# rajabala/Volumetric-Particles-For-Unity

Measured on AMD Instinct MI355X. Metric: Mvoxels/s filled + Msamples/s raymarched, 32³×32³ grid @1080p, higher is better.
Workload: dtype f32 compute / f16 voxel storage

## Files before the change

### volumetric-particles-for-unity_amd/csrc/api.cpp

```cpp
#include <cmath>
#include <cstdarg>
#include <cstdio>
#include <cstdlib>
#include <cstring>
#include <new>

#include "vpfx_internal.h"

thread_local std::string g_vp_create_error;

int vp_fail(vp_ctx* c, int code, const char* fmt, ...)
{
    char buf[512];
    va_list ap;
    va_start(ap, fmt);
    vsnprintf(buf, sizeof buf, fmt, ap);
    va_end(ap);
    if (c) c->err = buf; else g_vp_create_error = buf;
    return code;
}

namespace {

template <typename T>
// ... 224 lines not shown
    hipError_t e = hipGetDeviceCount(&ndev);
    if (e != hipSuccess || ndev < 1)
        return vp_fail(nullptr, VP_ERR_NO_DEVICE, "vp_create: no HIP device (%s); libvpfx has no CPU fallback",
                       e != hipSuccess ? hipGetErrorString(e) : "device count 0");
    int dev = cfg->device;
    if (dev < 0) { if (hipGetDevice(&dev) != hipSuccess) dev = 0; }
    if (dev >= ndev) return vp_fail(nullptr, VP_ERR_BAD_ARG, "vp_create: device %d of %d", dev, ndev);

    c = new (std::nothrow) vp_ctx();
    if (!c) return vp_fail(nullptr, VP_ERR_OOM, "vp_create: host allocation failed");
    c->cfg = *cfg;
    c->device = dev;
    if (cfg->multi_flags & VP_MULTI_TEST_HOOKS) { const char* hook = getenv("VPFX_TEST_CHAIN_TIMEOUT"); c->test_chain_timeout = hook && hook[0] == '1'; }
    { const char* sw = getenv("VPFX_RM_NO_SPACE_SKIP"); c->rm_space_skip = !sw ? 0 : sw[0] == '1' ? -1 : sw[0] == '0' ? 1 : 0; }
    { const char* sw = getenv("VPFX_RM_NO_BOX_CLIP"); c->rm_box_clip = !sw ? 0 : sw[0] == '1' ? -1 : sw[0] == '0' ? 1 : 0; }
#if VPFX_AB
    { const char* sw = getenv("VPFX_NO_ZPROFILE"); c->no_zprofile = sw && sw[0] == '1'; }
    { const char* sw = getenv("VPFX_RM_FLAT"); c->rm_flat = sw && sw[0] == '1'; }
    { const char* sw = getenv("VPFX_RM_XCD_AFFINE"); c->rm_xcd_affine = sw && sw[0] == '1'; }
#endif
    c->n3 = (size_t)cfg->num_mv[0] * cfg->num_mv[1] * cfg->num_mv[2];
    memset(c->L, 0, sizeof c->L); c->L[0] = c->L[5] = c->L[10] = c->L[15] = 1.f;
    c->h_mvPos = (float*)malloc(c->n3 * 3 * sizeof(float));
    int rc = VP_OK;
    auto fail = [&](int code) { g_vp_create_error = c->err; vp_destroy_single(c); return code; };
    if (!c->h_mvPos) { c->err = "vp_create: host allocation failed"; return fail(VP_ERR_OOM); }
    hl_build_grid(c);
    if ((rc = ensure_device(c))) return fail(rc);
    if (hipDeviceGetAttribute(&c->num_cus, hipDeviceAttributeMultiprocessorCount, dev) != hipSuccess || c->num_cus < 1) c->num_cus = 256;
    const size_t nxy = (size_t)cfg->num_mv[0] * cfg->num_mv[1];
    if ((rc = dev_alloc(c, &c->d_mvPos, c->n3 * 3)) || (rc = dev_alloc(c, &c->d_count, c->n3)) ||
        (rc = dev_alloc(c, &c->d_offsets, c->n3 + 1)) || (rc = dev_alloc(c, &c->d_cursor, c->n3)) ||
        (rc = dev_alloc(c, &c->d_brick_index, c->n3)) || (rc = dev_alloc(c, &c->d_occ_list, c->n3)) ||
        (rc = dev_alloc(c, &c->d_onecol, 2)) || (rc = dev_alloc(c, &c->d_work_counter, 1)) || (rc = dev_alloc(c, &c->d_meta, 1)) ||
        (rc = dev_alloc(c, &c->d_ord, c->n3)) || (rc = dev_alloc(c, &c->d_colcount, nxy)) || (rc = dev_alloc(c, &c->d_chain, lightmap_elems(c))) ||
        (rc = dev_alloc(c, (int4**)&c->d_scan_totals, (c->n3 + 1023) / 1024 + 1)) ||
        (rc = dev_alloc(c, &c->d_lightmap, lightmap_elems(c))) || (rc = dev_alloc(c, &c->d_rank, nxy)) ||
        (rc = dev_alloc(c, &c->d_image, image_elems(c))) || (rc = dev_alloc(c, &c->d_samples, 1)) ||
        (rc = dev_alloc(c, &c->d_zsamples, (size_t)VPFX_ZPROF_COPIES * cfg->num_mv[2])) ||
        (rc = dev_alloc(c, &c->d_tile_order, (size_t)rm_order_ints(rm_num_super_tiles(cfg->width, cfg->height)) + rm_num_super_tiles(cfg->width, cfg->height) + 8)))
        return fail(rc);
#if VPFX_AB
    {
        const int sgx = rm_super_tiles_x(cfg->width), sgy = rm_super_tiles_y(cfg->height), ns = sgx * sgy;
        int side = 1; while (side < sgx || side < sgy) side <<= 1;
        std::vector<int> curve; curve.reserve(ns);
        for (long long d = 0; d < (long long)side * side; ++d) {
            long long tt = d; int x = 0, y = 0;
// ... 24 lines not shown
}

VP_EXPORT void vp_destroy(vp_ctx* c)
{
    if (!c) return;
    if (c->multi) { multi_destroy(c); return; }
    vp_destroy_single(c);
}

void vp_destroy_single(vp_ctx* c)
{
    if (!c) return;
    (void)hipSetDevice(c->device);
    if (c->stream) (void)hipStreamSynchronize(c->stream); else (void)hipDeviceSynchronize();
    void* dev[] = {c->d_mvPos, c->d_raw, c->d_ws, c->d_rec, c->d_count, c->d_offsets, c->d_cursor, c->d_brick_index,
                   c->d_occ_list, c->d_ids_tmp, c->d_ids, c->d_onecol, c->d_work_counter, c->d_ord, c->d_colcount, c->d_chain, c->d_cube_u8, c->d_meta, c->d_scan_totals, c->d_bricks, c->d_dens_ao,
                   c->d_lightmap, c->d_cubequads, c->d_depthmap, c->d_occluders, c->d_mvtrans, c->d_brick_hit, c->d_rank, c->d_tile_order, c->d_tile_curve, c->d_image, c->d_scene_depth, c->d_samples, c->d_zsamples, c->d_cellinfo, c->d_occmask, c->d_slab_rect, c->d_mvbox[0], c->d_mvbox[1]};
    for (void* p : dev) if (p) (void)hipFree(p);
    mesh_free_all(c);
    device_emitters_orphan_all(c);
    particle_queries_free(c);
    if (c->h_chain_err) (void)hipHostFree(c->h_chain_err);
    if (c->h_meta_host) (void)hipHostFree(c->h_meta_host);
    if (c->copy_stream) { (void)hipStreamSynchronize(c->copy_stream); (void)hipStreamDestroy(c->copy_stream); }
    if (c->ev_image_ready) (void)hipEventDestroy(c->ev_image_ready);
    if (c->ev_image_copied) (void)hipEventDestroy(c->ev_image_copied);
    for (int s = 0; s < 4; ++s) for (int j = 0; j < 2; ++j) if (c->ev[s][j]) (void)hipEventDestroy(c->ev[s][j]);
    free(c->h_mvPos);
    delete c;
}

// ... 817 lines not shown
```

### volumetric-particles-for-unity_amd/csrc/bin.hip

```cpp
#include "vpfx_internal.h"
#include "mv_box.h"

#include <chrono>

namespace {

__device__ __forceinline__ float rd_f32(const uint8_t* p)
{
    uint32_t v = (uint32_t)p[0] | ((uint32_t)p[1] << 8) | ((uint32_t)p[2] << 16) | ((uint32_t)p[3] << 24);
    return __uint_as_float(v);
}

__device__ __forceinline__ void sincos_deg(float deg, float& s, float& c)
{
    const float k = rintf(deg * (1.0f / 90.0f));
    const float r = fmaf(-90.0f, k, deg);
    const float x = r * 0.017453292519943295f;
    const float z = x * x;
    const float sp = fmaf(fmaf(fmaf(-1.9515295891e-4f, z, 8.3321608736e-3f), z, -1.6666654611e-1f), z * x, x);
    const float cp = fmaf(fmaf(fmaf(2.443315711809948e-5f, z, -1.388731625493765e-3f), z, 4.166664568298827e-2f),
                          z * z, fmaf(-0.5f, z, 1.0f));
    switch (((int)k) & 3) {
    case 0: s = sp; c = cp; break;
    case 1: s = cp; c = -sp; break;
// ... 35 lines not shown
    for (int k = 0; k < 3; ++k) {
        const float rx = R[0 * 3 + k] * inv, ry = R[1 * 3 + k] * inv, rz = R[2 * 3 + k] * inv;
        out[k * 4 + 0] = rx; out[k * 4 + 1] = ry; out[k * 4 + 2] = rz;
        out[k * 4 + 3] = -((rx * wx + ry * wy) + rz * wz);
    }
    out[12] = life / life0;
    out[13] = 0.f; out[14] = 0.f; out[15] = 0.f;
    float4* dst = reinterpret_cast<float4*>(rec + 16 * (size_t)p);
    dst[0] = make_float4(out[0], out[1], out[2], out[3]);
    dst[1] = make_float4(out[4], out[5], out[6], out[7]);
    dst[2] = make_float4(out[8], out[9], out[10], out[11]);
    dst[3] = make_float4(out[12], out[13], out[14], out[15]);
}

#define BIN_LANES 32
template <int MODE>
__global__ void __launch_bounds__(256)
k_bin(const float4* __restrict__ ws4, int P, GridConsts g, const float* __restrict__ mvPos,
      int* __restrict__ count_or_cursor, const int* __restrict__ offsets, int* __restrict__ ids, float* __restrict__ rec,
      const DevMeta* __restrict__ ahead_meta, int ahead_cap)
{
    const long long t = (long long)blockIdx.x * 256 + threadIdx.x;
    const int p = (int)(t / BIN_LANES), sub = (int)(t % BIN_LANES);
    if (p >= P) return;
    if (MODE == 1 && ahead_meta && (unsigned)ahead_meta->pairs > (unsigned)ahead_cap) return;
    const float4 w = ws4[p];
    if (MODE == 0 && sub == 0) {
        float* r = rec + 16 * (size_t)p;
        const float dx = g.fwd[0] * g.one, dy = g.fwd[1] * g.one, dz = g.fwd[2] * g.one;
        r[13] = fmaf(r[2], dz, fmaf(r[1], dy, r[0] * dx));
        r[14] = fmaf(r[6], dz, fmaf(r[5], dy, r[4] * dx));
        r[15] = fmaf(r[10], dz, fmaf(r[9], dy, r[8] * dx));
    }
    if (!(fabsf(w.x) < INFINITY && fabsf(w.y) < INFINITY && fabsf(w.z) < INFINITY && fabsf(w.w) < INFINITY)) return;
    const float lx = ((g.Linv[0] * w.x + g.Linv[1] * w.y) + g.Linv[2] * w.z) + g.Linv[3];
    const float ly = ((g.Linv[4] * w.x + g.Linv[5] * w.y) + g.Linv[6] * w.z) + g.Linv[7];
    const float lz = ((g.Linv[8] * w.x + g.Linv[9] * w.y) + g.Linv[10] * w.z) + g.Linv[11];
    const float pix = (lx - g.lsO[0]) / g.s + (float)g.Nx * 0.5f;
    const float piy = (ly - g.lsO[1]) / g.s + (float)g.Ny * 0.5f;
    const float piz = (lz - g.lsO[2]) / g.s + (float)g.Nz * 0.5f;
    const float fe = (float)(int)rintf((w.w / 2.0f) / g.s);
    const int x0 = (int)fmaxf(0.f, pix - fe), x1 = (int)fminf((float)(g.Nx - 1), pix + fe);
    const int y0 = (int)fmaxf(0.f, piy - fe), y1 = (int)fminf((float)(g.Ny - 1), piy + fe);
    int z0 = (int)fmaxf(0.f, piz - fe), z1 = (int)fminf((float)(g.Nz - 1), piz + fe);
    if (MODE != 2) { z0 = max(z0, g.z0); z1 = min(z1, g.z1 - 1); }
    const float r = (w.w / 2.0f) / g.sb;
    const int nx = x1 - x0 + 1, ny = y1 - y0 + 1, nz = z1 - z0 + 1;
    if (nx <= 0 || ny <= 0 || nz <= 0) return;
    const int ncand = nx * ny * nz;
    for (int ci = sub; ci < ncand; ci += BIN_LANES) {
                const int xx = x0 + ci % nx, yy = y0 + (ci / nx) % ny, zz = z0 + ci / (nx * ny);
                const int mi = (zz * g.Ny + yy) * g.Nx + xx;
                const float mx = mvPos[3 * mi], my = mvPos[3 * mi + 1], mz = mvPos[3 * mi + 2];
                float r2 = r * r;
#pragma unroll
                for (int k = 0; k < 3; ++k) {
                    const float a = g.rowsb[k * 3], bq = g.rowsb[k * 3 + 1], cq = g.rowsb[k * 3 + 2];
                    const float t = -((a * mx + bq * my) + cq * mz);
                    const float m = ((a * w.x + bq * w.y) + cq * w.z) + t;
                    if (m < -0.5f) { const float d = m - (-0.5f); r2 -= d * d; }
                    else if (m > 0.5f) { const float d = m - 0.5f; r2 -= d * d; }
                }
                if (r2 > 0.f) {
                    if (MODE == 2) atomicAdd(&count_or_cursor[zz], 1);
                    else if (MODE == 0) atomicAdd(&count_or_cursor[mi], 1);
                    else { const int slot = atomicAdd(&count_or_cursor[mi], 1); ids[offsets[mi] + slot] = p; }
                }
            }
}

#define SCAN_TILE 1024
#define SCAN_DIRECT_TILES 4096
struct TileTotals { long long pairs; int occ, mx; };

__device__ __forceinline__ void block_scan3(long long& a, int& b, int& m, long long* sh )
{
    const int lane = threadIdx.x & 63, wv = threadIdx.x >> 6;
#pragma unroll
    for (int d = 1; d < 64; d <<= 1) {
        const long long ua = __shfl_up(a, d);
        const int ub = __shfl_up(b, d), um = __shfl_up(m, d);
        if (lane >= d) { a += ua; b += ub; m = max(m, um); }
    }
// ... 34 lines not shown
        const int t = base + threadIdx.x;
        const TileTotals tt = t < ntiles ? totals[t] : TileTotals{0, 0, 0};
        long long a = tt.pairs;
        int b = tt.occ, m = tt.mx;
        block_scan3(a, b, m, sh);
        const long long ca = s_carry[0];
        const int cb = (int)s_carry[1], cm = (int)s_carry[2];
        if (t < ntiles) totals[t] = TileTotals{ca + a - tt.pairs, cb + b - tt.occ, 0};
        __syncthreads();
        if (threadIdx.x == SCAN_TILE - 1) { s_carry[0] = ca + a; s_carry[1] = cb + b; s_carry[2] = max(cm, m); }
        __syncthreads();
    }
    if (threadIdx.x == 0) totals[ntiles] = TileTotals{s_carry[0], (int)s_carry[1], (int)s_carry[2]};
}

__device__ __forceinline__ void publish_totals(DevMeta* host_meta, const DevMeta& r, int seq)
{
    *host_meta = r;
    __hip_atomic_store(reinterpret_cast<int*>(host_meta + 1), seq, __ATOMIC_RELEASE, __HIP_MEMORY_SCOPE_SYSTEM);
}

__global__ void __launch_bounds__(SCAN_TILE)
k_scan_write(const int* __restrict__ count, int n3, int nxy, int z0, int z1, const TileTotals* __restrict__ totals, int ntiles,
             int prefixed, int* __restrict__ offsets, int* __restrict__ brick_index, int* __restrict__ occ_list, int* __restrict__ cursor,
             DevMeta* __restrict__ meta, DevMeta* __restrict__ host_meta, int seq, uint2* __restrict__ mvbox)
{
    __shared__ long long sh[48];
    __shared__ long long s_base[3];
    if (prefixed) {
        if (threadIdx.x == 0) { s_base[0] = totals[blockIdx.x].pairs; s_base[1] = totals[blockIdx.x].occ; s_base[2] = totals[ntiles].mx; }
    } else {
        long long pa = 0;
        int pb = 0, pm = 0;
        for (int t = threadIdx.x; t < ntiles; t += SCAN_TILE) {
            const TileTotals tt = totals[t];
            if (t < (int)blockIdx.x) { pa += tt.pairs; pb += tt.occ; }
            pm = max(pm, tt.mx);
        }
        block_scan3(pa, pb, pm, sh);
        if (threadIdx.x == SCAN_TILE - 1) { s_base[0] = pa; s_base[1] = pb; s_base[2] = pm; }
    }
    __syncthreads();
    const long long base_pairs = s_base[0];
// ... 6 lines not shown
    int b = occ ? 1 : 0, m = cnt;
    block_scan3(a, b, m, sh);
    if (i < n3) {
        offsets[i] = (int)(base_pairs + a - cnt);
        cursor[i] = 0;
        const int slot = base_occ + b - (occ ? 1 : 0);
        brick_index[i] = occ ? slot : -1;
        if (occ) occ_list[slot] = i;
        else mvbox[i] = make_uint2(VPFX_MVBOX_EMPTY_X, VPFX_MVBOX_EMPTY_Y);
    }
    if ((int)blockIdx.x == ntiles - 1 && threadIdx.x == SCAN_TILE - 1) {
        const long long total = base_pairs + a;
        offsets[n3] = (int)total;
        const DevMeta r{base_occ + b, total > 2147483647LL ? -1 : (int)total, gmax, 0};
        *meta = r;
        publish_totals(host_meta, r, seq);
    }
}

__global__ void __launch_bounds__(SCAN_TILE)
k_scan_small(const int* __restrict__ count, int n3, int nxy, int z0, int z1, int* __restrict__ offsets, int* __restrict__ brick_index,
             int* __restrict__ occ_list, int* __restrict__ cursor, int* __restrict__ ord, int* __restrict__ colcount,
             DevMeta* __restrict__ meta, DevMeta* __restrict__ host_meta, int seq, uint2* __restrict__ mvbox)
{
    __shared__ long long sh[48];
    __shared__ unsigned char s_occ[SCAN_TILE];
    const int i = threadIdx.x;
    const int cnt = i < n3 ? count[i] : 0;
    const int zz = i / nxy;
    const bool occ = cnt != 0 && zz >= z0 && zz < z1;
    s_occ[i] = occ ? 1 : 0;
// ... 14 lines not shown
        } else mvbox[i] = make_uint2(VPFX_MVBOX_EMPTY_X, VPFX_MVBOX_EMPTY_Y);
        if (i < nxy) {
            int n = 0;
            for (int z = z0; z < z1; ++z) n += s_occ[z * nxy + i];
            colcount[i] = n;
        }
    }
    if (i == SCAN_TILE - 1) {
        offsets[n3] = (int)a;
        const DevMeta r{b, a > 2147483647LL ? -1 : (int)a, m, 0};
        *meta = r;
        publish_totals(host_meta, r, seq);
    }
}

struct BoxConsts { float Rl[9]; float inv_sb; int nv; };
typedef unsigned short u16x2_t __attribute__((ext_vector_type(2)));

__device__ __forceinline__ void mv_boxes(const int* __restrict__ occ_list, const int* __restrict__ offsets, const int* __restrict__ in, int slot,
                                         const float4* __restrict__ ws4, const float* __restrict__ mvPos, const BoxConsts& bc, uint2* __restrict__ mvbox)
{
    const int lane = threadIdx.x & 63;
    const int mi = occ_list[slot];
    const int off = offsets[mi], n = offsets[mi + 1] - off;
    const float mvx = mvPos[3 * mi], mvy = mvPos[3 * mi + 1], mvz = mvPos[3 * mi + 2];
    MvBox acc = mv_box_empty();
    for (int i = lane; i < n; i += 64) {
        const float4 w = ws4[in[off + i]];
        MvBox b;
        if (mv_box_of_particle(w.x, w.y, w.z, w.w, mvx, mvy, mvz, bc.Rl, bc.inv_sb, bc.nv, b)) mv_box_union(acc, b);
// ... 2 lines not shown
            p2 = {(unsigned short)(255 - acc.hi[1]), (unsigned short)(255 - acc.hi[2])};
#pragma unroll
    for (int o = 32; o; o >>= 1) {
        p0 = __builtin_elementwise_min(p0, __builtin_bit_cast(u16x2_t, __shfl_xor(__builtin_bit_cast(int, p0), o)));
        p1 = __builtin_elementwise_min(p1, __builtin_bit_cast(u16x2_t, __shfl_xor(__builtin_bit_cast(int, p1), o)));
        p2 = __builtin_elementwise_min(p2, __builtin_bit_cast(u16x2_t, __shfl_xor(__builtin_bit_cast(int, p2), o)));
    }
    if (lane == 0) {
        const MvBox u{{(int)p0[0], (int)p0[1], (int)p1[0]}, {255 - (int)p1[1], 255 - (int)p2[0], 255 - (int)p2[1]}};
        uint32_t x, y;
        mv_box_pack(u, x, y);
        mvbox[mi] = make_uint2(x, y);
    }
}

#define SORT_CAP 4096
__global__ void __launch_bounds__(256)
k_sort_lists(const int* __restrict__ occ_list, const int* __restrict__ offsets, const int* __restrict__ in,
             int* __restrict__ out, DevMeta* __restrict__ meta, int ahead_cap, int nsort, const float4* __restrict__ ws4,
             const float* __restrict__ mvPos, BoxConsts bc, uint2* __restrict__ mvbox)
{
    __shared__ int s_ids[SORT_CAP];
    const int nbox = (nsort + 3) >> 2, sorter = (int)blockIdx.x - nbox;
    if (sorter < 0) {
        const int slot = (int)blockIdx.x * 4 + (int)(threadIdx.x >> 6);
        if (ahead_cap >= 0 ? (slot >= meta->occupied || (unsigned)meta->pairs > (unsigned)ahead_cap) : slot >= nsort) return;
        mv_boxes(occ_list, offsets, in, slot, ws4, mvPos, bc, mvbox);
        return;
    }
    if (ahead_cap >= 0 && (sorter >= meta->occupied || (unsigned)meta->pairs > (unsigned)ahead_cap)) return;
    const int mi = occ_list[sorter];
    const int off = offsets[mi], n = offsets[mi + 1] - off;
    if (n > SORT_CAP) {
        for (int i = threadIdx.x; i < n; i += 256) {
            const int v = in[off + i];
            int rank = 0;
            for (int j = 0; j < n; ++j) rank += (in[off + j] < v) ? 1 : 0;
            out[off + rank] = v;
        }
        if (threadIdx.x == 0) atomicAdd(&meta->unsorted_lists, 1);
// ... 31 lines not shown
int launch_extract(vp_ctx* c)
{
    if (c->P == 0) return VP_OK;
    hipLaunchKernelGGL(k_extract, dim3((c->P + 255) / 256), dim3(256), 0, c->stream,
                       c->d_raw, c->P, c->lay, c->psys, c->d_ws, c->d_rec);
    VP_HIP(hipGetLastError());
    return VP_OK;
}

int launch_z_histogram(vp_ctx* c, int* d_hist)
{
    const GridConsts& g = c->g;
    VP_HIP(hipMemsetAsync(d_hist, 0, (size_t)g.Nz * sizeof(int), c->stream));
    if (c->P > 0)
        hipLaunchKernelGGL(k_bin<2>, dim3((unsigned)(((size_t)c->P * BIN_LANES + 255) / 256)), dim3(256), 0, c->stream, c->d_ws, c->P, g, c->d_mvPos, d_hist,
                           (const int*)nullptr, (int*)nullptr, c->d_rec, (const DevMeta*)nullptr, 0);
    VP_HIP(hipGetLastError());
    return VP_OK;
}

int launch_bin(vp_ctx* c)
{
    const GridConsts& g = c->g;
    const int n3 = (int)c->n3, nxy = g.Nx * g.Ny;
    const unsigned nb = (unsigned)(((size_t)c->P * BIN_LANES + 255) / 256);
    VP_HIP(hipMemsetAsync(c->d_count, 0, c->n3 * sizeof(int), c->stream));
    VP_HIP(hipEventRecord(c->ev[0][0], c->stream));
    if (c->P > 0) {
        hipLaunchKernelGGL(k_bin<0>, dim3(nb), dim3(256), 0, c->stream, c->d_ws, c->P, g, c->d_mvPos, c->d_count,
                           (const int*)nullptr, (int*)nullptr, c->d_rec, (const DevMeta*)nullptr, 0);
    }
    const bool small = n3 <= SCAN_TILE;
    for (int i = 0; i < 2; ++i)
        if (!c->d_mvbox[i]) VP_HIP(hipMalloc((void**)&c->d_mvbox[i], c->n3 * sizeof(uint2)));
    uint2* box = c->d_mvbox[c->mvbox_cur ^ 1];
    c->mvbox_fresh = true;
    BoxConsts bc;
    for (int i = 0; i < 9; ++i) bc.Rl[i] = g.Rl[i];
    bc.inv_sb = g.inv_sb; bc.nv = g.nv;
    const int seq = ++c->bin_seq;
    if (c->bin_seq == 0x7fffffff) c->bin_seq = 0;
    if (small) {
        hipLaunchKernelGGL(k_scan_small, dim3(1), dim3(SCAN_TILE), 0, c->stream, c->d_count, n3, nxy, g.z0, g.z1, c->d_offsets, c->d_brick_index,
                           c->d_occ_list, c->d_cursor, c->d_ord, c->d_colcount, c->d_meta, c->d_meta_host, seq, box);
    } else {
        const int ntiles = (n3 + SCAN_TILE - 1) / SCAN_TILE;
        hipLaunchKernelGGL(k_scan_tiles, dim3(ntiles), dim3(SCAN_TILE), 0, c->stream, c->d_count, n3, nxy, g.z0, g.z1,
                           (TileTotals*)c->d_scan_totals);
        const int prefixed = ntiles > SCAN_DIRECT_TILES ? 1 : 0;
        if (prefixed) hipLaunchKernelGGL(k_scan_prefix, dim3(1), dim3(SCAN_TILE), 0, c->stream, (TileTotals*)c->d_scan_totals, ntiles);
        hipLaunchKernelGGL(k_scan_write, dim3(ntiles), dim3(SCAN_TILE), 0, c->stream, c->d_count, n3, nxy, g.z0, g.z1,
                           (const TileTotals*)c->d_scan_totals, ntiles, prefixed, c->d_offsets, c->d_brick_index, c->d_occ_list, c->d_cursor, c->d_meta,
                           c->d_meta_host, seq, box);
        hipLaunchKernelGGL(k_col_ordinal, dim3((nxy + 3) / 4), dim3(256), 0, c->stream, c->d_brick_index, nxy, g.z0, g.z1, c->d_ord, c->d_colcount);
    }
    const int ahead_cap = (int)(c->pairs_cap < 2147483647u ? c->pairs_cap : 2147483647u);
    const bool ahead = c->P > 0 && c->pairs_cap > 0, ahead_sort = ahead && small;
    if (ahead) {
        hipLaunchKernelGGL(k_bin<1>, dim3(nb), dim3(256), 0, c->stream, c->d_ws, c->P, g, c->d_mvPos, c->d_cursor,
                           (const int*)c->d_offsets, c->d_ids_tmp, c->d_rec, (const DevMeta*)c->d_meta, ahead_cap);
        if (ahead_sort)
            hipLaunchKernelGGL(k_sort_lists, dim3(n3 + (n3 + 3) / 4), dim3(256), 0, c->stream, c->d_occ_list, c->d_offsets,
                               (const int*)c->d_ids_tmp, c->d_ids, c->d_meta, ahead_cap, n3, (const float4*)c->d_ws, (const float*)c->d_mvPos, bc, box);
    }
    VP_HIP(hipGetLastError());
    {
        const volatile int* seq_word = reinterpret_cast<const volatile int*>(c->h_meta_host + 1);
        const auto t_begin = std::chrono::steady_clock::now();
        bool seen = false;
        for (unsigned spin = 0; !seen; ++spin) {
            if (__atomic_load_n(const_cast<const int*>(seq_word), __ATOMIC_ACQUIRE) == seq) { seen = true; break; }
            if ((spin & 1023u) == 1023u) {
                const hipError_t q = hipStreamQuery(c->stream);
                if (q == hipSuccess) break;
                if (q != hipErrorNotReady) return vp_fail(c, VP_ERR_HIP, "vp_bin: %s", hipGetErrorString(q));
                if (std::chrono::steady_clock::now() - t_begin > std::chrono::microseconds(400)) break;
            }
        }
        if (!seen) VP_HIP(hipStreamSynchronize(c->stream));
    }
    c->h_meta = *c->h_meta_host;
    if (c->h_meta.pairs < 0)
        return vp_fail(c, VP_ERR_UNSUPPORTED, "vp_bin: more than INT_MAX (particle, metavoxel) pairs; the CSR offsets are 32-bit");
    const size_t pairs = (size_t)c->h_meta.pairs;
    bool scattered = ahead, sorted = ahead_sort;
    if (pairs > c->pairs_cap) {
        if (c->d_ids) VP_HIP(hipFree(c->d_ids));
        if (c->d_ids_tmp) VP_HIP(hipFree(c->d_ids_tmp));
        c->d_ids = c->d_ids_tmp = nullptr;
        c->pairs_cap = pairs + pairs / 4 + 1024;
        VP_HIP(hipMalloc(&c->d_ids, c->pairs_cap * sizeof(int)));
        VP_HIP(hipMalloc(&c->d_ids_tmp, c->pairs_cap * sizeof(int)));
        scattered = sorted = false;
    }
    if (c->P > 0 && pairs > 0) {
        if (!scattered)
            hipLaunchKernelGGL(k_bin<1>, dim3(nb), dim3(256), 0, c->stream, c->d_ws, c->P, g, c->d_mvPos, c->d_cursor,
                               (const int*)c->d_offsets, c->d_ids_tmp, c->d_rec, (const DevMeta*)nullptr, 0);
        if (!sorted)
            hipLaunchKernelGGL(k_sort_lists, dim3(c->h_meta.occupied + (c->h_meta.occupied + 3) / 4), dim3(256), 0, c->stream, c->d_occ_list,
                               c->d_offsets, (const int*)c->d_ids_tmp, c->d_ids, c->d_meta, -1, c->h_meta.occupied, (const float4*)c->d_ws,
                               (const float*)c->d_mvPos, bc, box);
        VP_HIP(hipGetLastError());
    }
    VP_HIP(hipEventRecord(c->ev[0][1], c->stream));
    c->ev_valid[0] = true;
    return VP_OK;
}

namespace {
__global__ void __launch_bounds__(256)
k_mvbox_set(uint2* __restrict__ box, int n, uint2 v)
{
    const int i = blockIdx.x * 256 + threadIdx.x;
    if (i < n) box[i] = v;
}
}
// ... 24 lines not shown
```

### volumetric-particles-for-unity_amd/csrc/fill_kernels.h

```cpp
#pragma once
#include <cstdlib>
#include <type_traits>

#include "vpfx_internal.h"

#ifndef VPFX_FILL_PIPE_LDS
#define VPFX_FILL_PIPE_LDS 2
#endif
#ifndef VPFX_LDS_PITCH_128
#define VPFX_LDS_PITCH_128 136
#endif
#define VPFX_STR2(x) #x
#define VPFX_STR(x) VPFX_STR2(x)
#ifndef VPFX_PROBE
#define VPFX_PROBE 0
#endif
#if VPFX_PROBE && !VPFX_AB
#error "VPFX_PROBE builds produce wrong bricks on purpose: make EXTRA='-DVPFX_AB=1 -DVPFX_PROBE=n'"
#endif
#if VPFX_PROBE == 9
#ifdef VPFX_FILL_MAIN_TU
__device__ unsigned long long g_fill_prof[12];
extern "C" __attribute__((visibility("default"))) int vpfx_probe_read(unsigned long long* out, int reset)
{
// ... 697 lines not shown

int chain_begin(vp_ctx* c, const FillPtrs& P, int mode, FillChain& ch)
{
    const size_t lm = (size_t)c->g.Nx * c->g.nv * c->g.Ny * c->g.nv;
    if (mode == 0 && P.light_in) {
        if (P.light_in != P.light_out) VP_HIP(hipMemcpyAsync(P.light_out, P.light_in, lm * sizeof(float), hipMemcpyDeviceToDevice, c->stream));
    } else {
        int rc = launch_fill_value(c, P.light_out, lm, 1.0f, c->d_work_counter); if (rc) return rc;
    }
    if (mode == 0 && P.light_in) VP_HIP(hipMemsetAsync(c->d_work_counter, 0, sizeof(int), c->stream));
    const uint32_t span = (uint32_t)c->g.Nz + 1u;
    if (c->chain_seq >= 0xffffffffu / span - 1u) {
        VP_HIP(hipMemsetAsync(c->d_chain, 0, lm * sizeof(unsigned long long), c->stream));
        c->chain_seq = 0;
    }
    ch.words = c->d_chain; ch.ord = c->d_ord; ch.colcount = c->d_colcount; ch.occ_list = c->d_occ_list; ch.error = c->d_chain_err;
    const bool hook = c->test_chain_timeout;
    ch.spin_limit = hook ? 64u : VPFX_CHAIN_SPIN_LIMIT;
    ch.wait_bias = hook ? 0x40000000u : 0u;
    ch.tag_base = c->chain_seq * span;
    ++c->chain_seq;
    return VP_OK;
}

template <int NV, int MODE, int TAB, bool DONE, bool GEN = false>
int launch_fill_lds_variant(vp_ctx* c, const FillPtrs& P)
{
    const size_t bytes = cube_u8_bytes(c->cube_u8_S);
    auto kernel = k_fill_lds<NV, MODE, TAB, DONE, GEN>;
    { int rc = allow_big_lds(c, kernel, 160 * 1024 - 1024 ); if (rc) return rc; }
    const int TPC = GEN ? ((c->g.nv + 7) / 8) * ((c->g.nv + 7) / 8) : (NV / 8) * (NV / 8);
// ... 61 lines not shown
```

### volumetric-particles-for-unity_amd/csrc/vpfx_internal.h

```cpp
#pragma once

#include <hip/hip_runtime.h>
#include <stdint.h>
#include <string>
#include <vector>

#include "../../include/vpfx.h"

#define VP_EXPORT extern "C" __attribute__((visibility("default")))

#define VPFX_CFG_NO_LDS_CUBEMAP 1
#define VPFX_CFG_NO_GREY_BRICKS 1

struct MeshShape { int64_t first_vertex, n_vertices, first_triangle, n_triangles; };
struct MeshInstDev {
    float m[12];
    int32_t first_triangle, n_triangles;
    int32_t mirrored, pad;
};
struct MeshTri { float4 p0, p1, p2; };

struct GridConsts {
    int Nx, Ny, Nz, nv, b, z0, z1, pad0;
    float s, sb, one, inv_sb;
// ... 46 lines not shown
    float alpha_cutoff;
    int   box_clip;
    float inv_step_tex;
};
#define VPFX_RM_SKIP_RECTS 64

#ifndef VPFX_ZPROF_COPIES
#define VPFX_ZPROF_COPIES 64
#endif
struct RmHandoff {
    const uint8_t* t_in; int n_in; size_t plane;
    uint8_t* t_out0; uint8_t* t_out1;
    unsigned* zsamples;
};

struct DevMeta {
    int occupied;
    int pairs;
    int max_pairs;
    int unsorted_lists;
};

struct vp_multi;

struct vp_ctx {
    vp_config cfg{};
    vp_multi* multi = nullptr;
    bool test_chain_timeout = false;
    bool rm_xcd_affine = false;
    int* d_tile_curve = nullptr;
// ... 15 lines not shown
    size_t raw_cap = 0;
    uint8_t* d_raw = nullptr;
    float4* d_ws = nullptr;
    float* d_rec = nullptr;
    vp_particle_layout lay{};
    PsysConsts psys{};

    size_t n3 = 0;
    int* d_count = nullptr;
    int* d_offsets = nullptr;
    int* d_cursor = nullptr;
    int* d_brick_index = nullptr;
    int* d_occ_list = nullptr;
    int* d_ids_tmp = nullptr;
    int* d_ids = nullptr;
    size_t pairs_cap = 0;
    int* d_onecol = nullptr;
    DevMeta* d_meta = nullptr;
    DevMeta* h_meta_host = nullptr;
    DevMeta* d_meta_host = nullptr;
    void* d_scan_totals = nullptr;
    DevMeta h_meta{};
    int bin_seq = 0;

    uint2* d_bricks = nullptr;
    bool bricks_grey = false;
    size_t brick_cap = 0;
    float2* d_dens_ao = nullptr;
    size_t dens_cap = 0;
    float* d_lightmap = nullptr;
// ... 171 lines not shown
```

Baseline: 176,500.

## Record bin pairs in count pass, single-block scan, and cost-ordered fill

The count pass of binning now records (metavoxel, slot, particle) pairs into segmented buffers, so a cheap placement kernel can scatter ids without rerunning the full particle–metavoxel intersection test. A single-block scan kernel replaces the multi-kernel tiled scan and column-ordinal passes for mid-sized grids, which cuts launch count. The sort kernel also builds a per-layer fill order that ranks bricks by pair count, heaviest first, to balance the fill work. In exchange it adds an int4 pair buffer sized to capacity, extra atomics and ballots in the bin kernel, and fallback paths when a segment overflows.

```diff
diff --git a/volumetric-particles-for-unity_amd/csrc/api.cpp b/volumetric-particles-for-unity_amd/csrc/api.cpp
--- a/volumetric-particles-for-unity_amd/csrc/api.cpp
+++ b/volumetric-particles-for-unity_amd/csrc/api.cpp
@@ -262,6 +262,8 @@
     if (cfg->multi_flags & VP_MULTI_TEST_HOOKS) { const char* hook = getenv("VPFX_TEST_CHAIN_TIMEOUT"); c->test_chain_timeout = hook && hook[0] == '1'; }
     { const char* sw = getenv("VPFX_RM_NO_SPACE_SKIP"); c->rm_space_skip = !sw ? 0 : sw[0] == '1' ? -1 : sw[0] == '0' ? 1 : 0; }
     { const char* sw = getenv("VPFX_RM_NO_BOX_CLIP"); c->rm_box_clip = !sw ? 0 : sw[0] == '1' ? -1 : sw[0] == '0' ? 1 : 0; }
+    { const char* sw = getenv("VPFX_BIN_LEGACY"); c->bin_legacy = sw && sw[0] == '1'; }
+    { const char* sw = getenv("VPFX_FILL_RASTER_ORDER"); c->fill_raster_order = sw && sw[0] == '1'; }
 #if VPFX_AB
     { const char* sw = getenv("VPFX_NO_ZPROFILE"); c->no_zprofile = sw && sw[0] == '1'; }
     { const char* sw = getenv("VPFX_RM_FLAT"); c->rm_flat = sw && sw[0] == '1'; }
@@ -277,9 +279,9 @@
     if ((rc = ensure_device(c))) return fail(rc);
     if (hipDeviceGetAttribute(&c->num_cus, hipDeviceAttributeMultiprocessorCount, dev) != hipSuccess || c->num_cus < 1) c->num_cus = 256;
     const size_t nxy = (size_t)cfg->num_mv[0] * cfg->num_mv[1];
-    if ((rc = dev_alloc(c, &c->d_mvPos, c->n3 * 3)) || (rc = dev_alloc(c, &c->d_count, c->n3)) ||
+    if ((rc = dev_alloc(c, &c->d_mvPos, c->n3 * 3)) || (rc = dev_alloc(c, &c->d_count, c->n3 + VPFX_PAIR_CURSOR_INTS)) ||
         (rc = dev_alloc(c, &c->d_offsets, c->n3 + 1)) || (rc = dev_alloc(c, &c->d_cursor, c->n3)) ||
-        (rc = dev_alloc(c, &c->d_brick_index, c->n3)) || (rc = dev_alloc(c, &c->d_occ_list, c->n3)) ||
+        (rc = dev_alloc(c, &c->d_brick_index, c->n3)) || (rc = dev_alloc(c, &c->d_occ_list, c->n3)) || (rc = dev_alloc(c, &c->d_fill_order, c->n3)) ||
         (rc = dev_alloc(c, &c->d_onecol, 2)) || (rc = dev_alloc(c, &c->d_work_counter, 1)) || (rc = dev_alloc(c, &c->d_meta, 1)) ||
         (rc = dev_alloc(c, &c->d_ord, c->n3)) || (rc = dev_alloc(c, &c->d_colcount, nxy)) || (rc = dev_alloc(c, &c->d_chain, lightmap_elems(c))) ||
         (rc = dev_alloc(c, (int4**)&c->d_scan_totals, (c->n3 + 1023) / 1024 + 1)) ||
@@ -334,7 +336,7 @@
     (void)hipSetDevice(c->device);
     if (c->stream) (void)hipStreamSynchronize(c->stream); else (void)hipDeviceSynchronize();
     void* dev[] = {c->d_mvPos, c->d_raw, c->d_ws, c->d_rec, c->d_count, c->d_offsets, c->d_cursor, c->d_brick_index,
-                   c->d_occ_list, c->d_ids_tmp, c->d_ids, c->d_onecol, c->d_work_counter, c->d_ord, c->d_colcount, c->d_chain, c->d_cube_u8, c->d_meta, c->d_scan_totals, c->d_bricks, c->d_dens_ao,
+                   c->d_occ_list, c->d_fill_order, c->d_pair_rec, c->d_ids_tmp, c->d_ids, c->d_onecol, c->d_work_counter, c->d_ord, c->d_colcount, c->d_chain, c->d_cube_u8, c->d_meta, c->d_scan_totals, c->d_bricks, c->d_dens_ao,
                    c->d_lightmap, c->d_cubequads, c->d_depthmap, c->d_occluders, c->d_mvtrans, c->d_brick_hit, c->d_rank, c->d_tile_order, c->d_tile_curve, c->d_image, c->d_scene_depth, c->d_samples, c->d_zsamples, c->d_cellinfo, c->d_occmask, c->d_slab_rect, c->d_mvbox[0], c->d_mvbox[1]};
     for (void* p : dev) if (p) (void)hipFree(p);
     mesh_free_all(c);
diff --git a/volumetric-particles-for-unity_amd/csrc/bin.hip b/volumetric-particles-for-unity_amd/csrc/bin.hip
--- a/volumetric-particles-for-unity_amd/csrc/bin.hip
+++ b/volumetric-particles-for-unity_amd/csrc/bin.hip
@@ -73,25 +73,31 @@
 }
 
 #define BIN_LANES 32
+#define PAIR_SEGS 256
+#define PAIR_CURSOR_STRIDE 32
 template <int MODE>
 __global__ void __launch_bounds__(256)
 k_bin(const float4* __restrict__ ws4, int P, GridConsts g, const float* __restrict__ mvPos,
       int* __restrict__ count_or_cursor, const int* __restrict__ offsets, int* __restrict__ ids, float* __restrict__ rec,
-      const DevMeta* __restrict__ ahead_meta, int ahead_cap)
+      const DevMeta* __restrict__ ahead_meta, int ahead_cap, int4* __restrict__ pair_rec, unsigned* __restrict__ pair_cursor)
 {
     const long long t = (long long)blockIdx.x * 256 + threadIdx.x;
     const int p = (int)(t / BIN_LANES), sub = (int)(t % BIN_LANES);
-    if (p >= P) return;
+    bool live = p < P;
+    if (MODE != 3 && !live) return;
     if (MODE == 1 && ahead_meta && (unsigned)ahead_meta->pairs > (unsigned)ahead_cap) return;
-    const float4 w = ws4[p];
-    if (MODE == 0 && sub == 0) {
+    const float4 w = live ? ws4[p] : make_float4(0.f, 0.f, 0.f, 0.f);
+    if ((MODE == 0 || MODE == 3) && sub == 0 && live) {
         float* r = rec + 16 * (size_t)p;
         const float dx = g.fwd[0] * g.one, dy = g.fwd[1] * g.one, dz = g.fwd[2] * g.one;
         r[13] = fmaf(r[2], dz, fmaf(r[1], dy, r[0] * dx));
         r[14] = fmaf(r[6], dz, fmaf(r[5], dy, r[4] * dx));
         r[15] = fmaf(r[10], dz, fmaf(r[9], dy, r[8] * dx));
     }
-    if (!(fabsf(w.x) < INFINITY && fabsf(w.y) < INFINITY && fabsf(w.z) < INFINITY && fabsf(w.w) < INFINITY)) return;
+    if (!(fabsf(w.x) < INFINITY && fabsf(w.y) < INFINITY && fabsf(w.z) < INFINITY && fabsf(w.w) < INFINITY)) {
+        if (MODE != 3) return;
+        live = false;
+    }
     const float lx = ((g.Linv[0] * w.x + g.Linv[1] * w.y) + g.Linv[2] * w.z) + g.Linv[3];
     const float ly = ((g.Linv[4] * w.x + g.Linv[5] * w.y) + g.Linv[6] * w.z) + g.Linv[7];
     const float lz = ((g.Linv[8] * w.x + g.Linv[9] * w.y) + g.Linv[10] * w.z) + g.Linv[11];
@@ -105,11 +111,18 @@
     if (MODE != 2) { z0 = max(z0, g.z0); z1 = min(z1, g.z1 - 1); }
     const float r = (w.w / 2.0f) / g.sb;
     const int nx = x1 - x0 + 1, ny = y1 - y0 + 1, nz = z1 - z0 + 1;
-    if (nx <= 0 || ny <= 0 || nz <= 0) return;
-    const int ncand = nx * ny * nz;
-    for (int ci = sub; ci < ncand; ci += BIN_LANES) {
-                const int xx = x0 + ci % nx, yy = y0 + (ci / nx) % ny, zz = z0 + ci / (nx * ny);
-                const int mi = (zz * g.Ny + yy) * g.Nx + xx;
+    if (nx <= 0 || ny <= 0 || nz <= 0) {
+        if (MODE != 3) return;
+        live = false;
+    }
+    const int ncand = live ? nx * ny * nz : 0;
+    for (int ci = sub; MODE == 3 ? __builtin_amdgcn_ballot_w64(ci < ncand) != 0ull : ci < ncand; ci += BIN_LANES) {
+                bool hit = false;
+                int mi = 0, zz = 0;
+                if (ci < ncand) {
+                const int xx = x0 + ci % nx, yy = y0 + (ci / nx) % ny;
+                zz = z0 + ci / (nx * ny);
+                mi = (zz * g.Ny + yy) * g.Nx + xx;
                 const float mx = mvPos[3 * mi], my = mvPos[3 * mi + 1], mz = mvPos[3 * mi + 2];
                 float r2 = r * r;
 #pragma unroll
@@ -120,12 +133,43 @@
                     if (m < -0.5f) { const float d = m - (-0.5f); r2 -= d * d; }
                     else if (m > 0.5f) { const float d = m - 0.5f; r2 -= d * d; }
                 }
-                if (r2 > 0.f) {
+                hit = r2 > 0.f;
+                }
+                if (MODE == 3) {
+                    int slot = 0;
+                    if (hit) slot = atomicAdd(&count_or_cursor[mi], 1);
+                    const unsigned long long hits = __builtin_amdgcn_ballot_w64(hit);
+                    if (hits != 0ull) {
+                        const int lane = threadIdx.x & 63, leader = __builtin_ctzll(hits);
+                        unsigned base = 0u;
+                        const unsigned seg = blockIdx.x % PAIR_SEGS;
+                        if (lane == leader) base = atomicAdd(pair_cursor + seg * PAIR_CURSOR_STRIDE, (unsigned)__builtin_popcountll(hits));
+                        base = (unsigned)__shfl((int)base, leader);
+                        const unsigned at = base + (unsigned)__builtin_popcountll(hits & ((1ull << lane) - 1ull));
+                        if (hit && at < (unsigned)ahead_cap) pair_rec[(size_t)seg * (unsigned)ahead_cap + at] = make_int4(mi, slot, p, 0);
+                    }
+                } else if (hit) {
                     if (MODE == 2) atomicAdd(&count_or_cursor[zz], 1);
                     else if (MODE == 0) atomicAdd(&count_or_cursor[mi], 1);
                     else { const int slot = atomicAdd(&count_or_cursor[mi], 1); ids[offsets[mi] + slot] = p; }
                 }
             }
+}
+
+__device__ __forceinline__ int pair_segments_overflowed(const unsigned* __restrict__ pair_cursor, unsigned seg_cap)
+{
+    return __syncthreads_or(threadIdx.x < PAIR_SEGS && pair_cursor[threadIdx.x * PAIR_CURSOR_STRIDE] > seg_cap);
+}
+
+__global__ void __launch_bounds__(256)
+k_place(const int4* __restrict__ pair_rec, const unsigned* __restrict__ pair_cursor, unsigned seg_cap, const int* __restrict__ offsets,
+        int* __restrict__ ids)
+{
+    if (pair_segments_overflowed(pair_cursor, seg_cap)) return;
+    const unsigned t = blockIdx.x * 256u + threadIdx.x, seg = t / seg_cap;
+    if (seg >= PAIR_SEGS || t - seg * seg_cap >= pair_cursor[seg * PAIR_CURSOR_STRIDE]) return;
+    const int4 r = pair_rec[t];
+    ids[offsets[r.x] + r.y] = r.z;
 }
 
 #define SCAN_TILE 1024
@@ -190,19 +234,23 @@
     if (threadIdx.x == 0) totals[ntiles] = TileTotals{s_carry[0], (int)s_carry[1], (int)s_carry[2]};
 }
 
-__device__ __forceinline__ void publish_totals(DevMeta* host_meta, const DevMeta& r, int seq)
+__device__ __forceinline__ void publish_totals(DevMeta* host_meta, const DevMeta& r, int seq, int pair_overflow = 0)
 {
     *host_meta = r;
+    reinterpret_cast<int*>(host_meta + 1)[1] = pair_overflow;
     __hip_atomic_store(reinterpret_cast<int*>(host_meta + 1), seq, __ATOMIC_RELEASE, __HIP_MEMORY_SCOPE_SYSTEM);
 }
 
 __global__ void __launch_bounds__(SCAN_TILE)
 k_scan_write(const int* __restrict__ count, int n3, int nxy, int z0, int z1, const TileTotals* __restrict__ totals, int ntiles,
              int prefixed, int* __restrict__ offsets, int* __restrict__ brick_index, int* __restrict__ occ_list, int* __restrict__ cursor,
-             DevMeta* __restrict__ meta, DevMeta* __restrict__ host_meta, int seq, uint2* __restrict__ mvbox)
+             DevMeta* __restrict__ meta, DevMeta* __restrict__ host_meta, int seq, uint2* __restrict__ mvbox,
+             const unsigned* __restrict__ pair_cursor , unsigned seg_cap)
 {
     __shared__ long long sh[48];
     __shared__ long long s_base[3];
+    int pair_overflow = 0;
+    if ((int)blockIdx.x == ntiles - 1 && pair_cursor) pair_overflow = pair_segments_overflowed(pair_cursor, seg_cap);
     if (prefixed) {
         if (threadIdx.x == 0) { s_base[0] = totals[blockIdx.x].pairs; s_base[1] = totals[blockIdx.x].occ; s_base[2] = totals[ntiles].mx; }
     } else {
@@ -239,7 +287,7 @@
         offsets[n3] = (int)total;
         const DevMeta r{base_occ + b, total > 2147483647LL ? -1 : (int)total, gmax, 0};
         *meta = r;
-        publish_totals(host_meta, r, seq);
+        publish_totals(host_meta, r, seq, pair_overflow);
     }
 }
 
@@ -284,6 +332,87 @@
     }
 }
 
+#define SCAN_ONE_MAX 65536
+#define SCAN_ONE_MAX_NZ 128
+__global__ void __launch_bounds__(SCAN_TILE)
+k_scan_one(const int* __restrict__ count, int n3, int nxy, int z0, int z1, int* __restrict__ offsets, int* __restrict__ brick_index,
+           int* __restrict__ occ_list, int* __restrict__ cursor, int* __restrict__ ord, int* __restrict__ colcount,
+           DevMeta* __restrict__ meta, DevMeta* __restrict__ host_meta, int seq, uint2* __restrict__ mvbox,
+           const unsigned* __restrict__ pair_cursor , unsigned seg_cap)
+{
+    __shared__ long long sh[48];
+    __shared__ unsigned long long s_mask[SCAN_TILE];
+    __shared__ unsigned s_pb[SCAN_TILE];
+    __shared__ int s_ob[SCAN_TILE];
+    __shared__ long long s_sum[16];
+    const int tid = threadIdx.x, lane = tid & 63, wv = tid >> 6;
+    const int rounds = (n3 + SCAN_TILE - 1) / SCAN_TILE, nent = rounds * (SCAN_TILE / 64);
+    long long sum = 0;
+    int mx = 0;
+    const int pair_overflow = pair_cursor ? pair_segments_overflowed(pair_cursor, seg_cap) : 0;
+    for (int r = 0; r < rounds; ++r) {
+        const int i = r * SCAN_TILE + tid;
+        const int cnt = i < n3 ? count[i] : 0;
+        const int zz = i / nxy;
+        const bool occ = cnt != 0 && zz >= z0 && zz < z1;
+        sum += cnt;
+        mx = max(mx, cnt);
+        unsigned a = (unsigned)cnt;
+#pragma unroll
+        for (int d = 1; d < 64; d <<= 1) {
+            const unsigned u = (unsigned)__shfl_up((int)a, d);
+            if (lane >= d) a += u;
+        }
+        const unsigned long long m = __builtin_amdgcn_ballot_w64(occ);
+        if (i < n3) offsets[i] = (int)(a - (unsigned)cnt);
+        if (lane == 63) { const int j = r * (SCAN_TILE / 64) + wv; s_pb[j] = a; s_ob[j] = __builtin_popcountll(m); s_mask[j] = m; }
+    }
+    __syncthreads();
+    {
+        const unsigned tp = tid < nent ? s_pb[tid] : 0u;
+        const int to = tid < nent ? s_ob[tid] : 0;
+        long long a = tp;
+        int b = to, m = mx;
+        block_scan3(a, b, m, sh);
+        mx = m;
+        if (tid < nent) { s_pb[tid] = (unsigned)a - tp; s_ob[tid] = b - to; }
+#pragma unroll
+        for (int o = 32; o; o >>= 1) sum += __shfl_xor(sum, o);
+        if (lane == 0) s_sum[wv] = sum;
+    }
+    __syncthreads();
+    for (int r = 0; r < rounds; ++r) {
+        const int i = r * SCAN_TILE + tid, j = r * (SCAN_TILE / 64) + wv;
+        if (i >= n3) break;
+        const unsigned long long m = s_mask[j];
+        const bool occ = (m >> lane) & 1ull;
+        offsets[i] += (int)s_pb[j];
+        cursor[i] = 0;
+        const int slot = s_ob[j] + __builtin_popcountll(m & ((1ull << lane) - 1ull));
+        brick_index[i] = occ ? slot : -1;
+        if (occ) occ_list[slot] = i;
+        else mvbox[i] = make_uint2(VPFX_MVBOX_EMPTY_X, VPFX_MVBOX_EMPTY_Y);
+    }
+    for (int col = tid; col < nxy; col += SCAN_TILE) {
+        int n = 0;
+        for (int z = z0; z < z1; ++z) {
+            const int i = z * nxy + col;
+            if ((s_mask[i >> 6] >> (i & 63)) & 1ull) { ord[i] = n; ++n; }
+        }
+        colcount[col] = n;
+    }
+    if (tid == SCAN_TILE - 1) {
+        long long total = 0;
+#pragma unroll
+        for (int w = 0; w < 16; ++w) total += s_sum[w];
+        const int nocc = s_ob[nent - 1] + __builtin_popcountll(s_mask[nent - 1]);
+        offsets[n3] = (int)total;
+        const DevMeta r{nocc, total > 2147483647LL ? -1 : (int)total, mx, 0};
+        *meta = r;
+        publish_totals(host_meta, r, seq, pair_overflow);
+    }
+}
+
 struct BoxConsts { float Rl[9]; float inv_sb; int nv; };
 typedef unsigned short u16x2_t __attribute__((ext_vector_type(2)));
 
@@ -316,16 +445,59 @@
     }
 }
 
+#define ORDER_CAP 4096
+__device__ __forceinline__ void layer_order(const int* __restrict__ occ_list, const int* __restrict__ offsets, const int* __restrict__ brick_index,
+                                            int zz, int nxy, int* __restrict__ fill_order, unsigned* s_key , int* s_red )
+{
+    const int tid = threadIdx.x, first = zz * nxy;
+    if (tid == 0) { s_red[0] = 0x7fffffff; s_red[1] = 0; s_red[2] = 0; }
+    __syncthreads();
+    int lo = 0x7fffffff, n = 0, big = 0;
+    for (int i = tid; i < nxy; i += 256) {
+        const int bi = brick_index[first + i];
+        if (bi >= 0) { lo = min(lo, bi); ++n; big = max(big, offsets[first + i + 1] - offsets[first + i]); }
+    }
+    if (n) { atomicMin(&s_red[0], lo); atomicAdd(&s_red[1], n); atomicMax(&s_red[2], big); }
+    __syncthreads();
+    const int base = s_red[0], nocc = s_red[1];
+    if (nocc == 0) return;
+    if (nxy > ORDER_CAP || s_red[2] >= (1 << 20)) {
+        for (int i = tid; i < nxy; i += 256) { const int bi = brick_index[first + i]; if (bi >= 0) fill_order[bi] = first + i; }
+        return;
+    }
+    for (int i = tid; i < nxy; i += 256) {
+        const int bi = brick_index[first + i];
+        if (bi >= 0) s_key[bi - base] = ((unsigned)(offsets[first + i + 1] - offsets[first + i]) << 12) | (unsigned)(ORDER_CAP - 1 - (bi - base));
+    }
+    if (tid < 4 && (nocc & ~3) + tid >= nocc && (nocc & ~3) + tid < ((nocc + 3) & ~3)) s_key[(nocc & ~3) + tid] = 0u;
+    __syncthreads();
+    const uint4* k4 = reinterpret_cast<const uint4*>(s_key);
+    const int n4 = (nocc + 3) >> 2;
+    for (int k = tid; k < nocc; k += 256) {
+        const unsigned v = s_key[k];
+        int rank = 0;
+        for (int j = 0; j < n4; ++j) { const uint4 q = k4[j]; rank += (q.x > v) + (q.y > v) + (q.z > v) + (q.w > v); }
+        fill_order[base + rank] = occ_list[base + k];
+    }
+}
+
 #define SORT_CAP 4096
 __global__ void __launch_bounds__(256)
 k_sort_lists(const int* __restrict__ occ_list, const int* __restrict__ offsets, const int* __restrict__ in,
              int* __restrict__ out, DevMeta* __restrict__ meta, int ahead_cap, int nsort, const float4* __restrict__ ws4,
-             const float* __restrict__ mvPos, BoxConsts bc, uint2* __restrict__ mvbox)
-{
-    __shared__ int s_ids[SORT_CAP];
-    const int nbox = (nsort + 3) >> 2, sorter = (int)blockIdx.x - nbox;
+             const float* __restrict__ mvPos, BoxConsts bc, uint2* __restrict__ mvbox, int nlayer, int z0, int nxy,
+             const int* __restrict__ brick_index, int* __restrict__ fill_order)
+{
+    __shared__ __attribute__((aligned(16))) int s_ids[SORT_CAP];
+    __shared__ int s_red[3];
+    if ((int)blockIdx.x < nlayer) {
+        layer_order(occ_list, offsets, brick_index, z0 + (int)blockIdx.x, nxy, fill_order, reinterpret_cast<unsigned*>(s_ids), s_red);
+        return;
+    }
+    const int bid = (int)blockIdx.x - nlayer;
+    const int nbox = (nsort + 3) >> 2, sorter = bid - nbox;
     if (sorter < 0) {
-        const int slot = (int)blockIdx.x * 4 + (int)(threadIdx.x >> 6);
+        const int slot = bid * 4 + (int)(threadIdx.x >> 6);
         if (ahead_cap >= 0 ? (slot >= meta->occupied || (unsigned)meta->pairs > (unsigned)ahead_cap) : slot >= nsort) return;
         mv_boxes(occ_list, offsets, in, slot, ws4, mvPos, bc, mvbox);
         return;
@@ -387,7 +559,7 @@
     VP_HIP(hipMemsetAsync(d_hist, 0, (size_t)g.Nz * sizeof(int), c->stream));
     if (c->P > 0)
         hipLaunchKernelGGL(k_bin<2>, dim3((unsigned)(((size_t)c->P * BIN_LANES + 255) / 256)), dim3(256), 0, c->stream, c->d_ws, c->P, g, c->d_mvPos, d_hist,
-                           (const int*)nullptr, (int*)nullptr, c->d_rec, (const DevMeta*)nullptr, 0);
+                           (const int*)nullptr, (int*)nullptr, c->d_rec, (const DevMeta*)nullptr, 0, (int4*)nullptr, (unsigned*)nullptr);
     VP_HIP(hipGetLastError());
     return VP_OK;
 }
@@ -397,13 +569,22 @@
     const GridConsts& g = c->g;
     const int n3 = (int)c->n3, nxy = g.Nx * g.Ny;
     const unsigned nb = (unsigned)(((size_t)c->P * BIN_LANES + 255) / 256);
-    VP_HIP(hipMemsetAsync(c->d_count, 0, c->n3 * sizeof(int), c->stream));
+    const bool small = n3 <= SCAN_TILE;
+    const int ahead_cap = (int)(c->pairs_cap < 2147483647u ? c->pairs_cap : 2147483647u);
+    const bool ahead = c->P > 0 && c->pairs_cap > 0, ahead_sort = ahead && small;
+    const unsigned seg_cap = (unsigned)(ahead_cap / PAIR_SEGS);
+    const bool record = ahead && !small && !c->bin_legacy && c->d_pair_rec && seg_cap > 0;
+    unsigned* pair_cursor = reinterpret_cast<unsigned*>(c->d_count + c->n3);
+    VP_HIP(hipMemsetAsync(c->d_count, 0, (c->n3 + (record ? VPFX_PAIR_CURSOR_INTS : 0)) * sizeof(int), c->stream));
     VP_HIP(hipEventRecord(c->ev[0][0], c->stream));
     if (c->P > 0) {
-        hipLaunchKernelGGL(k_bin<0>, dim3(nb), dim3(256), 0, c->stream, c->d_ws, c->P, g, c->d_mvPos, c->d_count,
-                           (const int*)nullptr, (int*)nullptr, c->d_rec, (const DevMeta*)nullptr, 0);
-    }
-    const bool small = n3 <= SCAN_TILE;
+        if (record)
+            hipLaunchKernelGGL(k_bin<3>, dim3(nb), dim3(256), 0, c->stream, c->d_ws, c->P, g, c->d_mvPos, c->d_count,
+                               (const int*)nullptr, (int*)nullptr, c->d_rec, (const DevMeta*)nullptr, (int)seg_cap, c->d_pair_rec, pair_cursor);
+        else
+            hipLaunchKernelGGL(k_bin<0>, dim3(nb), dim3(256), 0, c->stream, c->d_ws, c->P, g, c->d_mvPos, c->d_count,
+                               (const int*)nullptr, (int*)nullptr, c->d_rec, (const DevMeta*)nullptr, 0, (int4*)nullptr, (unsigned*)nullptr);
+    }
     for (int i = 0; i < 2; ++i)
         if (!c->d_mvbox[i]) VP_HIP(hipMalloc((void**)&c->d_mvbox[i], c->n3 * sizeof(uint2)));
     uint2* box = c->d_mvbox[c->mvbox_cur ^ 1];
@@ -416,6 +597,10 @@
     if (small) {
         hipLaunchKernelGGL(k_scan_small, dim3(1), dim3(SCAN_TILE), 0, c->stream, c->d_count, n3, nxy, g.z0, g.z1, c->d_offsets, c->d_brick_index,
                            c->d_occ_list, c->d_cursor, c->d_ord, c->d_colcount, c->d_meta, c->d_meta_host, seq, box);
+    } else if (!c->bin_legacy && n3 <= SCAN_ONE_MAX && g.Nz <= SCAN_ONE_MAX_NZ) {
+        hipLaunchKernelGGL(k_scan_one, dim3(1), dim3(SCAN_TILE), 0, c->stream, c->d_count, n3, nxy, g.z0, g.z1, c->d_offsets, c->d_brick_index,
+                           c->d_occ_list, c->d_cursor, c->d_ord, c->d_colcount, c->d_meta, c->d_meta_host, seq, box,
+                           record ? (const unsigned*)pair_cursor : (const unsigned*)nullptr, seg_cap);
     } else {
         const int ntiles = (n3 + SCAN_TILE - 1) / SCAN_TILE;
         hipLaunchKernelGGL(k_scan_tiles, dim3(ntiles), dim3(SCAN_TILE), 0, c->stream, c->d_count, n3, nxy, g.z0, g.z1,
@@ -424,17 +609,20 @@
         if (prefixed) hipLaunchKernelGGL(k_scan_prefix, dim3(1), dim3(SCAN_TILE), 0, c->stream, (TileTotals*)c->d_scan_totals, ntiles);
         hipLaunchKernelGGL(k_scan_write, dim3(ntiles), dim3(SCAN_TILE), 0, c->stream, c->d_count, n3, nxy, g.z0, g.z1,
                            (const TileTotals*)c->d_scan_totals, ntiles, prefixed, c->d_offsets, c->d_brick_index, c->d_occ_list, c->d_cursor, c->d_meta,
-                           c->d_meta_host, seq, box);
+                           c->d_meta_host, seq, box, record ? (const unsigned*)pair_cursor : (const unsigned*)nullptr, seg_cap);
         hipLaunchKernelGGL(k_col_ordinal, dim3((nxy + 3) / 4), dim3(256), 0, c->stream, c->d_brick_index, nxy, g.z0, g.z1, c->d_ord, c->d_colcount);
     }
-    const int ahead_cap = (int)(c->pairs_cap < 2147483647u ? c->pairs_cap : 2147483647u);
-    const bool ahead = c->P > 0 && c->pairs_cap > 0, ahead_sort = ahead && small;
     if (ahead) {
-        hipLaunchKernelGGL(k_bin<1>, dim3(nb), dim3(256), 0, c->stream, c->d_ws, c->P, g, c->d_mvPos, c->d_cursor,
-                           (const int*)c->d_offsets, c->d_ids_tmp, c->d_rec, (const DevMeta*)c->d_meta, ahead_cap);
+        if (record)
+            hipLaunchKernelGGL(k_place, dim3((unsigned)(((size_t)seg_cap * PAIR_SEGS + 255) / 256)), dim3(256), 0, c->stream, (const int4*)c->d_pair_rec,
+                               (const unsigned*)pair_cursor, seg_cap, (const int*)c->d_offsets, c->d_ids_tmp);
+        else
+            hipLaunchKernelGGL(k_bin<1>, dim3(nb), dim3(256), 0, c->stream, c->d_ws, c->P, g, c->d_mvPos, c->d_cursor,
+                               (const int*)c->d_offsets, c->d_ids_tmp, c->d_rec, (const DevMeta*)c->d_meta, ahead_cap, (int4*)nullptr, (unsigned*)nullptr);
         if (ahead_sort)
             hipLaunchKernelGGL(k_sort_lists, dim3(n3 + (n3 + 3) / 4), dim3(256), 0, c->stream, c->d_occ_list, c->d_offsets,
-                               (const int*)c->d_ids_tmp, c->d_ids, c->d_meta, ahead_cap, n3, (const float4*)c->d_ws, (const float*)c->d_mvPos, bc, box);
+                               (const int*)c->d_ids_tmp, c->d_ids, c->d_meta, ahead_cap, n3, (const float4*)c->d_ws, (const float*)c->d_mvPos, bc, box,
+                               0, 0, nxy, (const int*)nullptr, (int*)nullptr);
     }
     VP_HIP(hipGetLastError());
     {
@@ -457,23 +645,31 @@
         return vp_fail(c, VP_ERR_UNSUPPORTED, "vp_bin: more than INT_MAX (particle, metavoxel) pairs; the CSR offsets are 32-bit");
     const size_t pairs = (size_t)c->h_meta.pairs;
     bool scattered = ahead, sorted = ahead_sort;
+    if (record && c->h_meta_host[1].pairs != 0) scattered = false;
     if (pairs > c->pairs_cap) {
         if (c->d_ids) VP_HIP(hipFree(c->d_ids));
         if (c->d_ids_tmp) VP_HIP(hipFree(c->d_ids_tmp));
+        if (c->d_pair_rec) VP_HIP(hipFree(c->d_pair_rec));
         c->d_ids = c->d_ids_tmp = nullptr;
+        c->d_pair_rec = nullptr;
         c->pairs_cap = pairs + pairs / 4 + 1024;
         VP_HIP(hipMalloc(&c->d_ids, c->pairs_cap * sizeof(int)));
         VP_HIP(hipMalloc(&c->d_ids_tmp, c->pairs_cap * sizeof(int)));
+        if (!small && !c->bin_legacy) VP_HIP(hipMalloc((void**)&c->d_pair_rec, c->pairs_cap * sizeof(int4)));
         scattered = sorted = false;
     }
+    c->fill_order_valid = false;
     if (c->P > 0 && pairs > 0) {
         if (!scattered)
             hipLaunchKernelGGL(k_bin<1>, dim3(nb), dim3(256), 0, c->stream, c->d_ws, c->P, g, c->d_mvPos, c->d_cursor,
-                               (const int*)c->d_offsets, c->d_ids_tmp, c->d_rec, (const DevMeta*)nullptr, 0);
-        if (!sorted)
-            hipLaunchKernelGGL(k_sort_lists, dim3(c->h_meta.occupied + (c->h_meta.occupied + 3) / 4), dim3(256), 0, c->stream, c->d_occ_list,
+                               (const int*)c->d_offsets, c->d_ids_tmp, c->d_rec, (const DevMeta*)nullptr, 0, (int4*)nullptr, (unsigned*)nullptr);
+        if (!sorted) {
+            const int nlayer = (!small && !c->fill_raster_order && c->d_fill_order) ? g.z1 - g.z0 : 0;
+            hipLaunchKernelGGL(k_sort_lists, dim3(nlayer + c->h_meta.occupied + (c->h_meta.occupied + 3) / 4), dim3(256), 0, c->stream, c->d_occ_list,
                                c->d_offsets, (const int*)c->d_ids_tmp, c->d_ids, c->d_meta, -1, c->h_meta.occupied, (const float4*)c->d_ws,
-                               (const float*)c->d_mvPos, bc, box);
+                               (const float*)c->d_mvPos, bc, box, nlayer, g.z0, nxy, (const int*)c->d_brick_index, c->d_fill_order);
+            c->fill_order_valid = nlayer > 0;
+        }
         VP_HIP(hipGetLastError());
     }
     VP_HIP(hipEventRecord(c->ev[0][1], c->stream));
diff --git a/volumetric-particles-for-unity_amd/csrc/fill_kernels.h b/volumetric-particles-for-unity_amd/csrc/fill_kernels.h
--- a/volumetric-particles-for-unity_amd/csrc/fill_kernels.h
+++ b/volumetric-particles-for-unity_amd/csrc/fill_kernels.h
@@ -735,7 +735,7 @@
         VP_HIP(hipMemsetAsync(c->d_chain, 0, lm * sizeof(unsigned long long), c->stream));
         c->chain_seq = 0;
     }
-    ch.words = c->d_chain; ch.ord = c->d_ord; ch.colcount = c->d_colcount; ch.occ_list = c->d_occ_list; ch.error = c->d_chain_err;
+    ch.words = c->d_chain; ch.ord = c->d_ord; ch.colcount = c->d_colcount; ch.occ_list = c->fill_order_valid ? c->d_fill_order : c->d_occ_list; ch.error = c->d_chain_err;
     const bool hook = c->test_chain_timeout;
     ch.spin_limit = hook ? 64u : VPFX_CHAIN_SPIN_LIMIT;
     ch.wait_bias = hook ? 0x40000000u : 0u;
diff --git a/volumetric-particles-for-unity_amd/csrc/vpfx_internal.h b/volumetric-particles-for-unity_amd/csrc/vpfx_internal.h
--- a/volumetric-particles-for-unity_amd/csrc/vpfx_internal.h
+++ b/volumetric-particles-for-unity_amd/csrc/vpfx_internal.h
@@ -84,6 +84,7 @@
     unsigned* zsamples;
 };
 
+#define VPFX_PAIR_CURSOR_INTS (256 * 32)
 struct DevMeta {
     int occupied;
     int pairs;
@@ -129,6 +130,11 @@
     int* d_occ_list = nullptr;
     int* d_ids_tmp = nullptr;
     int* d_ids = nullptr;
+    int4* d_pair_rec = nullptr;
+    int* d_fill_order = nullptr;
+    bool fill_order_valid = false;
+    bool bin_legacy = false;
+    bool fill_raster_order = false;
     size_t pairs_cap = 0;
     int* d_onecol = nullptr;
     DevMeta* d_meta = nullptr;
```

New measurement: 175,100. No clear change (-0.8%).
